# wedevxer/CUDA-AcceleratedVectorDatabaseEngine

Hardware: AMD Instinct MI355X
Metric: QPS + p99 latency, 10M×768D IVF-Flat k=10 nprobe=32, 1/2/4/8 MI355X (higher is better)
Workload: dtype fp32; 1 GPU; 10M x 768D IVF-Flat L2, nlist 4096, nprobe 32, batch 64, k 10; nvec=10000000, dim=768, nlist=4096, nprobe=32, batch=64, k=10, train_vectors=100000, parallelism=single GPU; 3 batches in flight

## Files before the change

cuda-acceleratedvectordatabaseengine_amd/csrc/screen.hip:

```cpp
#pragma clang fp contract(off)

#include <hip/hip_runtime.h>

#include <algorithm>
#include <stdexcept>
#include <cfloat>
#include <type_traits>

#include "kernels.hpp"
#include "scan_common.hpp"
#include "wave_topk.hpp"

namespace vdbk {

typedef __bf16 bf16x8 __attribute__((ext_vector_type(8)));
typedef float f32x4 __attribute__((ext_vector_type(4)));
typedef uint32_t u32x4 __attribute__((ext_vector_type(4)));
typedef int i32x4 __attribute__((ext_vector_type(4)));

constexpr float kScreenHuge = 1125899906842624.0f;
constexpr int kRing = 512;
#ifndef VDB_SCREEN_EXACT_PIPE
#define VDB_SCREEN_EXACT_PIPE 4
#endif
constexpr int kExactPipe = VDB_SCREEN_EXACT_PIPE;
#ifndef VDB_SCREEN_EXACT_PIPE_END
#define VDB_SCREEN_EXACT_PIPE_END 8
#endif
constexpr int kExactPipeEnd = VDB_SCREEN_EXACT_PIPE_END;
#ifndef VDB_SCREEN_DIAG
#define VDB_SCREEN_DIAG 0
#endif

__device__ __forceinline__ uint32_t bf16_bits(float f) {
    const uint32_t b = __float_as_uint(f);
    const uint32_t ex = b & 0x7F800000u;
    if (ex == 0) return 0u;
    if (ex == 0x7F800000u) return 0x7FC0u;
    return (b + 0x7FFFu + ((b >> 16) & 1u)) >> 16;
}
__device__ __forceinline__ float bf16_val(uint32_t h) { return __uint_as_float(h << 16); }

__device__ __forceinline__ uint4 pack_bf16x8(const float4 lo, const float4 hi) {
    uint4 r;
    r.x = bf16_bits(lo.x) | (bf16_bits(lo.y) << 16);
    r.y = bf16_bits(lo.z) | (bf16_bits(lo.w) << 16);
    r.z = bf16_bits(hi.x) | (bf16_bits(hi.y) << 16);
    r.w = bf16_bits(hi.z) | (bf16_bits(hi.w) << 16);
    return r;
}

__device__ __forceinline__ float4 resid(const float4 x, const float4 c) {
    return make_float4((float)((double)x.x - c.x), (float)((double)x.y - c.y), (float)((double)x.z - c.z),
                       (float)((double)x.w - c.w));
}

__device__ __forceinline__ float ru(double v) { return __double2float_ru(v * (1.0 + 0x1p-30)); }

__global__ __launch_bounds__(256) void ivf_screen_build(const float4* __restrict__ arena, uint64_t blocks,
                                                        uint32_t d4, const uint32_t* __restrict__ block_list,
                                                        const float* __restrict__ cent_rm, uint4* __restrict__ shadow,
                                                        float* __restrict__ rows, float4* __restrict__ meta) {
    const int lane = lane_id();
    const uint32_t dp = d4 * 4, ks = dp / 32;
    for (uint64_t b = (uint64_t)blockIdx.x * 4 + wave_index(); b < blocks; b += (uint64_t)gridDim.x * 4) {
        const float4* blk = arena + b * d4 * 64;
        const float4* cen = (const float4*)(cent_rm + (size_t)block_list[b] * dp);
        const uint64_t slot = b * 64 + lane;
        float4* row = rows ? (float4*)(rows + slot * dp) : nullptr;
        double x2 = 0.0, b2 = 0.0, e2 = 0.0;
        bool huge = false;
        for (uint32_t t = 0; t < d4; ++t) {
            const float4 x = blk[(size_t)t * 64 + lane];
            const float4 c = cen[t];
            if (rows) row[t] = x;
            const float xv[4] = {x.x, x.y, x.z, x.w}, cv[4] = {c.x, c.y, c.z, c.w};
#pragma unroll
            for (int i = 0; i < 4; ++i) {
                const double bd = (double)xv[i] - (double)cv[i];
                const double ed = bd - (double)bf16_val(bf16_bits((float)bd));
                huge |= !(fabs(bd) <= (double)kScreenHuge) || !(fabsf(xv[i]) <= kScreenHuge);
                x2 += (double)xv[i] * xv[i];
                b2 += bd * bd;
                e2 += ed * ed;
            }
        }
        meta[slot] = huge ? make_float4(__builtin_inff(), __builtin_inff(), __builtin_inff(), __builtin_inff())
                          : make_float4((float)b2, ru(sqrt(b2)), ru(sqrt(e2)), ru(sqrt(x2)));
        uint4* sh = shadow + b * (uint64_t)d4 * 32;
        const int vv = lane & 15, h = lane >> 4;
        for (uint32_t s = 0; s < ks; ++s) {
            const float4 c0 = cen[8 * s + 2 * h], c1 = cen[8 * s + 2 * h + 1];
            for (int vt = 0; vt < 4; ++vt) {
                const float4 lo = blk[(size_t)(8 * s + 2 * h) * 64 + 16 * vt + vv];
                const float4 hi = blk[(size_t)(8 * s + 2 * h + 1) * 64 + 16 * vt + vv];
                sh[((size_t)s * 4 + vt) * 64 + lane] = pack_bf16x8(resid(lo, c0), resid(hi, c1));
            }
        }
    }
}

template <int M>
__global__ __launch_bounds__(256) void ivf_screen_pairs(const float* __restrict__ q, uint32_t BP, uint32_t P,
                                                        const uint32_t* __restrict__ probes,
                                                        const float* __restrict__ cent_rm, uint32_t dp,
                                                        uint16_t* __restrict__ qres, float4* __restrict__ pst,
                                                        uint32_t* __restrict__ thr4, uint32_t* __restrict__ scnt,
                                                        uint32_t* __restrict__ ovf, uint32_t* __restrict__ counters,
                                                        uint32_t* __restrict__ ubcnt) {
    chain_prio();
    const int lane = lane_id();
    for (uint32_t e = blockIdx.x * blockDim.x + threadIdx.x; e < 4 * BP; e += gridDim.x * blockDim.x) thr4[e] = kThrInf;
    if (scnt)
        for (uint32_t e = blockIdx.x * blockDim.x + threadIdx.x; e < BP; e += gridDim.x * blockDim.x) {
            scnt[e] = 0u;
            ovf[e] = 0u;
            ubcnt[e] = 0u;
            if (e == 0) counters[kCtrCand] = counters[kCtrOvf] = counters[kCtrReal] = 0u;
        }
    for (uint32_t i = blockIdx.x * 4 + wave_index(); i < BP; i += gridDim.x * 4) {
        const float* qr = q + (size_t)(i / P) * dp;
        const float* cr = cent_rm + (size_t)probes[i] * dp;
        double a2 = 0.0, f2 = 0.0, c2 = 0.0, qc = 0.0;
        bool huge = false;
        for (uint32_t d = lane; d < dp; d += 64) {
            const float qv = qr[d], cv = cr[d];
            const double ad = M == kL2 ? (double)qv - (double)cv : (double)qv;
            const uint32_t h = bf16_bits((float)ad);
            qres[(size_t)i * dp + d] = (uint16_t)h;
            const double fd = ad - (double)bf16_val(h);
            huge |= !(fabs(ad) <= (double)kScreenHuge) || !(fabsf(qv) <= kScreenHuge) || !(fabsf(cv) <= kScreenHuge);
            a2 += ad * ad;
            f2 += fd * fd;
            c2 += (double)cv * cv;
            qc += (double)qv * cv;
        }
        for (int m = 32; m >= 1; m >>= 1) {
            a2 += __shfl_xor(a2, m);
            f2 += __shfl_xor(f2, m);
            c2 += __shfl_xor(c2, m);
            qc += __shfl_xor(qc, m);
        }
        huge = __ballot(huge) != 0;
        if (lane == 0) {
            const float inf = __builtin_inff();
            if (huge) pst[i] = make_float4(inf, inf, inf, inf);
            else if (M == kL2) pst[i] = make_float4((float)a2, ru(sqrt(a2)), ru(sqrt(f2)), 0.0f);
            else pst[i] = make_float4((float)qc, ru(sqrt(a2)), ru(sqrt(f2)), ru(sqrt(c2)));
        }
    }
}

__device__ __forceinline__ float i8_scale(float mx) { return mx > 0.0f ? mx * (1.0f / 127.0f) * (1.0f + 0x1p-20f) : 0.0f; }
__device__ __forceinline__ int i8_q(float r, float inv) { return max(-127, min(127, (int)rintf(r * inv))); }

__global__ __launch_bounds__(256) void ivf_screen_build_i8(const float4* __restrict__ arena, uint64_t blocks,
                                                           uint32_t d4, const uint32_t* __restrict__ block_list,
                                                           const float* __restrict__ cent_rm, uint4* __restrict__ shadow,
                                                           float* __restrict__ rows, float4* __restrict__ meta,
                                                           float* __restrict__ sscale) {
    const int lane = lane_id();
// ... 415 lines not shown
    char* base = (char*)slds + screen_item_lds(a.k, wq) + (size_t)wv * screen_wave_lds(a.k);
    uint64_t* tk_i = (uint64_t*)base;
    float* tk_d = (float*)(base + (size_t)16 * a.k * 8);
    float* kdl = tk_d + 16 * a.k;
    uint32_t* s_thr_w = (uint32_t*)(kdl + 16);
    uint32_t* ring = s_thr_w + 16;
    __shared__ uint32_t s_next, s_seg[2];
    __shared__ uint32_t s_thr[32];
    const int lane = lane_id();

    auto drain_narrow = [&]() {
        const uint32_t n_narrow = a.counters[0];
        for (;;) {
            uint32_t idx = 0;
            if (lane == 0) idx = atomicAdd(&a.work[0], 1u);
            idx = __builtin_amdgcn_readfirstlane(idx);
            if (idx >= n_narrow) break;
            ScanItem it = a.items[idx];
            it.list = __builtin_amdgcn_readfirstlane(it.list);
            it.seg = __builtin_amdgcn_readfirstlane(it.seg);
            it.pair_start = __builtin_amdgcn_readfirstlane(it.pair_start);
            it.npairs = __builtin_amdgcn_readfirstlane(it.npairs);
            if (lane < (int)it.npairs) s_thr_w[lane] = a.thr[it.pair_start + lane];
            __builtin_amdgcn_fence(__ATOMIC_RELEASE, "wavefront");
            screen_segment<M, KD>(a, it, 0, (int)it.npairs, it.seg, tk_d, tk_i, kdl, s_thr_w, ring, true, nullptr,
                                  it.seg);
            screen_partials(a, it, 0, (int)it.npairs, it.seg, tk_d, tk_i, true);
        }
    };

    const uint32_t n_wide = a.counters[3];
    uint32_t stride = a.wide_stride;
    if (stride > 1 && n_wide % stride == 0) stride = stride == 40009u ? 40013u : 40009u;
    if (a.fused && blockIdx.x + a.fused >= gridDim.x) drain_narrow();
    for (;;) {
        if (threadIdx.x == 0) s_next = atomicAdd(&a.work[1], 1u);
        __syncthreads();
        const uint32_t b = s_next;
        if (b >= n_wide) break;
        const uint32_t item = stride > 1 ? (uint32_t)(((uint64_t)b * stride) % n_wide) : b;
        ScanItem it = a.items_w[item];
        it.list = __builtin_amdgcn_readfirstlane(it.list);
        it.seg = __builtin_amdgcn_readfirstlane(it.seg);
        it.pair_start = __builtin_amdgcn_readfirstlane(it.pair_start);
        it.npairs = __builtin_amdgcn_readfirstlane(it.npairs);
        const int nq = (int)it.npairs;
        if (threadIdx.x < 2) s_seg[threadIdx.x] = 0;
        if (threadIdx.x < (uint32_t)nq) s_thr[threadIdx.x] = a.thr[it.pair_start + threadIdx.x];
        for (uint32_t e = threadIdx.x; e < (uint32_t)nq * a.k; e += blockDim.x) {
            it_d[e] = __builtin_inff();
            it_i[e] = kNoId;
        }
        if (threadIdx.x < (uint32_t)nq) {
            it_kd[threadIdx.x] = __builtin_inff();
            it_lock[threadIdx.x] = 0u;
        }
        __syncthreads();
        const uint32_t seg_vectors = a.seg_blocks * 64;
        const uint32_t nseg = (a.count[it.list] + seg_vectors - 1) / seg_vectors;
        const uint32_t seg0 = it.seg * a.segs_item, seg1 = min(nseg, seg0 + a.segs_item);
        const bool split = nq > 16;
        const uint32_t half = split ? wv >> 1 : 0u;
        const int nq0 = split ? (nq + 1) / 2 : nq;
        const int q0 = half ? nq0 : 0, nqh = half ? nq - nq0 : nq0;
        const int ko = q0 * (int)a.k;
        for (;;) {
            uint32_t sg = 0;
            if (lane == 0) sg = atomicAdd(&s_seg[half], 1u);
            sg = seg0 + __builtin_amdgcn_readfirstlane(sg);
            if (sg >= seg1) break;
            screen_segment<M, KD>(a, it, q0, nqh, sg, it_d + ko, it_i + ko, it_kd + q0, s_thr + q0, ring, false,
                                  it_lock + q0, it.seg);
            screen_partials(a, it, q0, nqh, sg, it_d + ko, it_i + ko, false);
        }
        __syncthreads();
        if ((wv & 1) == 0 && (wv == 0 || split)) screen_partials(a, it, q0, nqh, seg0, it_d + ko, it_i + ko, true);
    }
    if (a.fused) drain_narrow();
}


__device__ __forceinline__ void block_sort64(float (&u)[4]) {
    const int l = lane_id() & 15;
    bitonic64_step<2, 1>(u, l);
    bitonic64_step<4, 2>(u, l), bitonic64_step<4, 1>(u, l);
    bitonic64_step<8, 4>(u, l), bitonic64_step<8, 2>(u, l), bitonic64_step<8, 1>(u, l);
    bitonic64_step<16, 8>(u, l), bitonic64_step<16, 4>(u, l), bitonic64_step<16, 2>(u, l), bitonic64_step<16, 1>(u, l);
    bitonic64_step<32, 16>(u, l), bitonic64_step<32, 8>(u, l), bitonic64_step<32, 4>(u, l);
    bitonic64_step<32, 2>(u, l), bitonic64_step<32, 1>(u, l);
    bitonic64_step<64, 32>(u, l), bitonic64_step<64, 16>(u, l), bitonic64_step<64, 8>(u, l);
    bitonic64_step<64, 4>(u, l), bitonic64_step<64, 2>(u, l), bitonic64_step<64, 1>(u, l);
}
__device__ __forceinline__ void merge_sorted64(float (&rl)[4], const float (&u)[4]) {
    const int l = lane_id() & 15;
#pragma unroll
    for (int v = 0; v < 4; ++v) {
        const float rv = __uint_as_float((uint32_t)__builtin_amdgcn_mov_dpp((int)__float_as_uint(u[3 - v]), 0x140, 0xF,
                                                                            0xF, false));
        rl[v] = fminf(rl[v], rv);
    }
    bitonic64_step<64, 32>(rl, l), bitonic64_step<64, 16>(rl, l), bitonic64_step<64, 8>(rl, l);
    bitonic64_step<64, 4>(rl, l), bitonic64_step<64, 2>(rl, l), bitonic64_step<64, 1>(rl, l);
}
__device__ __forceinline__ float row_elem(const float (&u)[4], int e) {
    const int v = e & 3;
    const float x = v == 0 ? u[0] : v == 1 ? u[1] : v == 2 ? u[2] : u[3];
    return __shfl(x, (lane_id() & ~15) + (e >> 2));
}

struct CandChunk {
    uint32_t base = 0, left = 0;
    uint32_t next = 0;
    uint32_t real = 0;
    bool pending = false;
};
__device__ __forceinline__ void pad_cand(const ScanArgs& a, uint32_t base, uint32_t n) {
    for (uint32_t i = (uint32_t)lane_id(); i < n; i += 64)
        if (base + i < a.cand_cap) a.cand[base + i] = make_uint4(~0u, 0u, 0u, ~0u);
}
__device__ __forceinline__ void finish_cand(const ScanArgs& a, CandChunk& cc) {
    pad_cand(a, cc.base, cc.left);
    if (cc.pending) pad_cand(a, cc.next, kCandChunk);
    if (cc.real && lane_id() == 0) atomicAdd(a.ccount + (kCtrReal - kCtrCand), cc.real);
    cc.left = 0;
    cc.real = 0;
    cc.pending = false;
}

template <int M, int KD, int NG, bool I8, bool W2>
__device__ __forceinline__ void collect_segment(const ScanArgs& a, const ScanItem it, const int q0, const int nq,
                                                const uint32_t seg, float4* rl_lds, uint32_t* s_thr,
                                                const float4* s_pst, const float* s_qsc, float4* s_mt, float* s_vs,
                                                const uint32_t residue, CandChunk& cc) {
    const int lane = lane_id();
    const uint32_t dp = a.dp, ks = dp >> (I8 ? 6 : 5);
    const uint32_t count = a.count[it.list];
    const uint32_t seg_vectors = a.seg_blocks * 64;
    const uint64_t b0 = a.block_off[it.list] + (uint64_t)seg * a.seg_blocks;
    const uint32_t v0 = seg * seg_vectors;
    const uint32_t nv = min(count - v0, seg_vectors);
    const uint32_t nb = (nv + 63) >> 6;
    const int k = (int)a.k, kq = ((int)a.k + 3) / 4;
    const uint32_t* pairs = a.sorted_pair + it.pair_start + q0;
    const float cm = (float)(4 * dp + 16) * 0x1.02p-24f;
    const float cr = (float)(dp + 2) * 0x1.02p-24f;
    const float cu = 0x1.02p-23f;
    auto pair_of = [&](int g) -> uint32_t {
        const uint32_t pr = pairs[g];
        return (pr >> 16) * a.P + (pr & 0xFFFFu);
    };
    const uint4* qa_row[NG];
#pragma unroll
    for (int gg = 0; gg < NG; ++gg)
        qa_row[gg] = (const uint4*)((const char*)a.qres + (size_t)pair_of(min(16 * gg + (lane & 15), nq - 1)) * dp *
                                                              (I8 ? 1 : 2)) +
                     (lane >> 4);
    uint32_t collected = 0;
    float gthr[NG][4], gq4[NG][4];
#pragma unroll
    for (int gg = 0; gg < NG; ++gg)
#pragma unroll
        for (int r = 0; r < 4; ++r) gthr[gg][r] = gq4[gg][r] = __builtin_inff();
    const uint32_t thr_every = W2 ? a.thr_every : 1u;
    const uint32_t spl = it.pair_start + q0 + min(lane & (16 * NG - 1), nq - 1);

    const uint4* sp = a.shadow + b0 * (uint64_t)ks * 256 + lane;
    uint4 xa[KD][4], qa[NG][KD];
#pragma unroll
    for (int u = 0; u < KD; ++u) {
#pragma unroll
        for (int vt = 0; vt < 4; ++vt) xa[u][vt] = ld_nt_u4(sp + (size_t)(u * 4 + vt) * 64);
#pragma unroll
        for (int gg = 0; gg < NG; ++gg) qa[gg][u] = qa_row[gg][4 * (u % ks)];
    }
    using AccT = std::conditional_t<I8, i32x4, f32x4>;
    for (uint32_t j = 0; j < nb; ++j) {
        const uint64_t mslot = (b0 + j) * 64 + lane;
        const float4 mt_l = a.meta[mslot];
        float vs_l = 0.0f;
        if constexpr (I8) vs_l = a.sscale[mslot];
        const bool thr_now = j % thr_every == 0;
        uint32_t gt_l = 0u;
        uint4 t4_l = make_uint4(0u, 0u, 0u, 0u);
        if (thr_now) {
            gt_l = a.thr[spl];
            t4_l = *(const uint4*)(a.thr4 + (size_t)spl * 4);
        }
        const bool reserve = !cc.pending && cc.left < kCandChunk / 2;
        uint32_t reply = 0;
        if (reserve && lane == 0) reply = atomicAdd(a.ccount, kCandChunk);
        AccT acc[NG][4];
#pragma unroll
        for (int gg = 0; gg < NG; ++gg)
#pragma unroll
            for (int vt = 0; vt < 4; ++vt) acc[gg][vt] = AccT{0, 0, 0, 0};
        for (uint32_t s0 = 0; s0 < ks; s0 += KD) {
            static_for<0, KD>([&](auto uu) {
                constexpr int u = decltype(uu)::value;
#pragma unroll
                for (int gg = 0; gg < NG; ++gg) {
                    if constexpr (I8) {
                        const i32x4 A = as_i32x4(qa[gg][u]);
#pragma unroll
                        for (int vt = 0; vt < 4; ++vt)
                            acc[gg][vt] =
                                __builtin_amdgcn_mfma_i32_16x16x64_i8(A, as_i32x4(xa[u][vt]), acc[gg][vt], 0, 0, 0);
                    } else {
                        const bf16x8 A = as_bf16x8(qa[gg][u]);
#pragma unroll
                        for (int vt = 0; vt < 4; ++vt)
                            acc[gg][vt] =
                                __builtin_amdgcn_mfma_f32_16x16x32_bf16(A, as_bf16x8(xa[u][vt]), acc[gg][vt], 0, 0, 0);
                    }
                }
                const uint64_t nxt = (uint64_t)j * ks + s0 + u + KD;
#pragma unroll
                for (int vt = 0; vt < 4; ++vt) xa[u][vt] = ld_nt_u4(sp + (nxt * 4 + vt) * 64);
#pragma unroll
                for (int gg = 0; gg < NG; ++gg) qa[gg][u] = qa_row[gg][4 * ((s0 + u + KD) % ks)];
            });
        }
        s_mt[lane] = mt_l;
        if constexpr (I8) s_vs[lane] = vs_l;
        if (reserve) {
            cc.next = __builtin_amdgcn_readfirstlane(reply);
            cc.pending = true;
        }
        float gthr_l = 0.0f, gq4_l = 0.0f;
        if (thr_now) {
            const float th4 =
                fmaxf(fmaxf(ord_dec(t4_l.x), ord_dec(t4_l.y)), fmaxf(ord_dec(t4_l.z), ord_dec(t4_l.w)));
            gthr_l = fminf(ord_dec(gt_l), th4);
            gq4_l = ord_dec(residue == 0 ? t4_l.x : residue == 1 ? t4_l.y : residue == 2 ? t4_l.z : t4_l.w);
        }
        __builtin_amdgcn_fence(__ATOMIC_RELEASE, "wavefront");
#pragma unroll
        for (int gg = 0; gg < NG; ++gg) {
            const int g0 = 16 * gg;
            float ubv[4][4];
            float4 pst[4];
            float qsc[4];
#pragma unroll
            for (int r = 0; r < 4; ++r) {
                const int gc = min(g0 + 4 * (lane >> 4) + r, nq - 1);
                pst[r] = s_pst[gc];
                if constexpr (I8) qsc[r] = s_qsc[gc];
            }
#pragma unroll
            for (int vt = 0; vt < 4; ++vt) {
                const float4 mt = s_mt[16 * vt + (lane & 15)];
                float vsc = 0.0f;
                if constexpr (I8) vsc = s_vs[16 * vt + (lane & 15)];
                const bool valid = j * 64 + 16 * vt + (lane & 15) < nv;
#pragma unroll
                for (int r = 0; r < 4; ++r) {
                    float dot;
                    if constexpr (I8) dot = (float)acc[gg][vt][r] * (qsc[r] * vsc);
                    else dot = acc[gg][vt][r];
                    const float4 ps = pst[r];
                    const float approx = M == kL2 ? (ps.x + mt.x) - 2.0f * dot : -(ps.x + dot);
                    const float an = ps.y + ps.z, bn = mt.y + mt.z;
                    const float cs = an * mt.z + ps.z * bn + ps.z * mt.z;
                    float del;
                    if (M == kL2) {
                        const float rest = 2.0f * (cs + cm * (an * bn)) + cu * (ps.x + mt.x + fabsf(approx));
                        del = rest + cr * (fabsf(approx) + rest);
                    } else {
                        del = cs + cm * (an * bn) + cr * (ps.y * mt.w) + cu * (ps.y * ps.w + an * bn + fabsf(approx));
                    }
                    del = del * 1.001f + 1e-30f;
                    const float ub = approx + del;
                    if constexpr (I8) acc[gg][vt][r] = __float_as_int(approx - del);
                    else acc[gg][vt][r] = approx - del;
                    ubv[r][vt] = valid && ub == ub ? ub : __builtin_inff();
                }
            }
            float th[4], pub_t[4], pub_q[4];
#pragma unroll
            for (int r = 0; r < 4; ++r) {
                const int g = g0 + 4 * (lane >> 4) + r;
                const int gc = min(g, nq - 1);
                float4* rlp = rl_lds + (gg * 4 + r) * 64 + lane;
                const float4 rv = *rlp;
                float rl[4] = {rv.x, rv.y, rv.z, rv.w};
                float tw = row_elem(rl, k - 1), tq = row_elem(rl, kq - 1);
                if (thr_now) {
                    const float gn = __shfl(gthr_l, gc), qn = __shfl(gq4_l, gc);
                    if constexpr (W2) {
                        gthr[gg][r] = fminf(gthr[gg][r], gn);
                        gq4[gg][r] = fminf(gq4[gg][r], qn);
                    } else {
                        gthr[gg][r] = gn;
                        gq4[gg][r] = qn;
                    }
                }
                const float cur = fminf(gthr[gg][r], ord_dec(s_thr[gc]));
                const float bmin = fminf(fminf(ubv[r][0], ubv[r][1]), fminf(ubv[r][2], ubv[r][3]));
                if (__ballot(bmin < fminf(tw, cur))) {
                    block_sort64(ubv[r]);
                    merge_sorted64(rl, ubv[r]);
                    *rlp = make_float4(rl[0], rl[1], rl[2], rl[3]);
                    tw = row_elem(rl, k - 1);
                    tq = row_elem(rl, kq - 1);
                }
                pub_t[r] = tw < cur ? tw : __builtin_inff();
                pub_q[r] = tq < gq4[gg][r] ? tq : __builtin_inff();
                gthr[gg][r] = fminf(gthr[gg][r], tw);
                gq4[gg][r] = fminf(gq4[gg][r], tq);
                th[r] = g < nq ? fminf(tw, cur) : -__builtin_inff();
            }
            {
                const int lq = lane & 15, src = 16 * (lq >> 2), rs = lq & 3;
                float pt = __builtin_inff(), pq = __builtin_inff();
#pragma unroll
                for (int r = 0; r < 4; ++r) {
                    const float t = __shfl(pub_t[r], src), q = __shfl(pub_q[r], src);
                    if (rs == r) pt = t, pq = q;
                }
                if ((lane >> 4) == gg && g0 + lq < nq) {
                    if (pt < __builtin_inff()) {
                        atomicMin(&s_thr[g0 + lq], ord_enc(pt));
                        atomicMin(a.thr + spl, ord_enc(pt));
                    }
                    if (pq < __builtin_inff()) atomicMin(a.thr4 + (size_t)spl * 4 + residue, ord_enc(pq));
                }
            }
            auto lbv = [&](int vt, int r) -> float {
                if constexpr (I8) return __int_as_float(acc[gg][vt][r]);
                else return acc[gg][vt][r];
            };
            auto is_cand = [&](int vt, int r) {
                return j * 64 + 16 * vt + (lane & 15) < nv && g0 + 4 * (lane >> 4) + r < nq && !(lbv(vt, r) > th[r]);
            };
            uint32_t tot = 0;
#pragma unroll
            for (int vt = 0; vt < 4; ++vt)
#pragma unroll
                for (int r = 0; r < 4; ++r) tot += (uint32_t)__popcll(__ballot(is_cand(vt, r)));
            if (tot) {
                uint32_t cb0, cn0, cb1 = 0;
                if (tot <= cc.left) {
                    cb0 = cc.base;
                    cn0 = tot;
                    cc.base += tot;
                    cc.left -= tot;
                } else if (tot > kCandChunk) {
                    uint32_t v = 0;
                    if (lane == 0) v = atomicAdd(a.ccount, tot);
                    cb0 = __builtin_amdgcn_readfirstlane(v);
                    cn0 = tot;
                } else {
                    cb0 = cc.base;
                    cn0 = cc.left;
                    uint32_t v = 0;
                    if (cc.pending) {
                        cb1 = cc.next;
                        cc.pending = false;
                    } else {
                        if (lane == 0) v = atomicAdd(a.ccount, kCandChunk);
                        cb1 = __builtin_amdgcn_readfirstlane(v);
                    }
                    cc.base = cb1 + (tot - cn0);
                    cc.left = kCandChunk - (tot - cn0);
                }
                collected += tot;
                cc.real += tot;
                uint32_t rank = 0;
#pragma unroll
                for (int vt = 0; vt < 4; ++vt) {
#pragma unroll
                    for (int r = 0; r < 4; ++r) {
                        const bool c = is_cand(vt, r);
                        const uint64_t mm = __ballot(c);
                        if (c) {
                            const uint32_t rk = rank + __builtin_amdgcn_mbcnt_hi(
                                                           (uint32_t)(mm >> 32), __builtin_amdgcn_mbcnt_lo((uint32_t)mm, 0u));
                            const uint32_t idx = rk < cn0 ? cb0 + rk : cb1 + (rk - cn0);
                            const uint32_t spi = it.pair_start + q0 + g0 + 4 * (lane >> 4) + r;
                            const uint32_t slot = (uint32_t)((b0 + j) * 64 + 16 * vt + (lane & 15));
                            if (idx < a.cand_cap)
                                a.cand[idx] = make_uint4(spi, slot, __float_as_uint(lbv(vt, r)), 0u);
                            else {
                                a.ovf[spi] = 1u;
                                a.ccount[kCtrOvf - kCtrCand] = 1u;
                            }
                        }
                        rank += (uint32_t)__popcll(mm);
                    }
                }
            }
        }
    }
    if (a.mstats && lane == 0) {
        atomicAdd(&a.mstats[0], (unsigned long long)collected);
        atomicAdd(&a.mstats[1], (unsigned long long)nb);
    }
}

__device__ __forceinline__ void overflow_item(const ScanArgs& a, uint32_t pair_start, uint32_t npairs, uint32_t t0,
                                              uint32_t nt) {
    for (uint32_t t = t0; t < npairs; t += nt) a.ovf[pair_start + t] = 1u;
    if (t0 == 0) a.ccount[kCtrOvf - kCtrCand] = 1u;
}

__device__ __forceinline__ void reset_rl(float4* rl_lds, int rows) {
    const int lane = lane_id();
    const float inf = __builtin_inff();
    for (int r = 0; r < rows; ++r) rl_lds[r * 64 + lane] = make_float4(inf, inf, inf, inf);
}

__device__ __forceinline__ void contribute_rl(const ScanArgs& a, const ScanItem it, const int q0, const int nq,
                                              const float4* rl_lds) {
    const int lane = lane_id();
    const int k = (int)a.k;
    for (int r = 0; r < (nq + 15) / 16 * 4; ++r) {
        const int g = 16 * (r >> 2) + 4 * (lane >> 4) + (r & 3);
        const uint32_t spi = it.pair_start + q0 + min(g, nq - 1);
        uint32_t slot = 0;
        if ((lane & 15) == 0 && g < nq) slot = atomicAdd(&a.ubcnt[spi], 1u);
        slot = __shfl(slot, lane & ~15);
        const float4 rv = rl_lds[r * 64 + lane];
        const float rl[4] = {rv.x, rv.y, rv.z, rv.w};
        if (g < nq && slot < (uint32_t)kUbLists) {
            float* dst = a.ublist + ((size_t)spi * kUbLists + slot) * k;
#pragma unroll
            for (int v = 0; v < 4; ++v) {
                const int e = 4 * (lane & 15) + v;
                if (e < k) dst[e] = rl[v];
            }
        }
    }
}

__device__ __forceinline__ void put_stamp(const ScanArgs& a, uint64_t w0, uint64_t t0, uint64_t w3) {
    const uint32_t i = atomicAdd((unsigned int*)a.stamps, 1u);
    if (i < a.stamps_cap) {
        unsigned long long* r = a.stamps + 2 + (size_t)i * 4;
        r[0] = ((uint64_t)a.stamp_batch << 40) | w0;
        r[1] = t0;
        r[2] = wall_clock64();
        r[3] = w3;
    }
}

template <int M, int KD, bool W2, bool I8>
__global__ __launch_bounds__(256, W2 ? 1 : 2) void ivf_screen_collect(ScanArgs a) {
    __shared__ uint32_t s_next, s_seg;
    __shared__ uint32_t s_thr[32];
    __shared__ uint32_t s_thr_w[4][16];
    __shared__ float4 s_rl[4][8 * 64];
    __shared__ float4 s_pst[32], s_pst_w[4][16];
    __shared__ float s_qsc[32], s_qsc_w[4][16];
    __shared__ float4 s_mt[4][64];
    __shared__ float s_vs[4][64];
    const uint32_t wv = wave_index();
    const int lane = lane_id();
    float4* rl = s_rl[wv];
    CandChunk cc;
    auto pair_stats = [&](uint32_t ps, uint32_t t, float4* dp4, float* dsc) {
        const uint32_t pr = a.sorted_pair[ps + t];
        const uint32_t pi = (pr >> 16) * a.P + (pr & 0xFFFFu);
        dp4[t] = a.pst[pi];
        if (I8) dsc[t] = a.qscale[pi];
    };

    auto drain_narrow = [&]() {
        const uint32_t n_narrow = a.counters[0];
        for (;;) {
            uint32_t idx = 0;
            if (lane == 0) idx = atomicAdd(&a.work[0], 1u);
            idx = __builtin_amdgcn_readfirstlane(idx);
            if (idx >= n_narrow) break;
            ScanItem it = a.items[idx];
            it.list = __builtin_amdgcn_readfirstlane(it.list);
            it.seg = __builtin_amdgcn_readfirstlane(it.seg);
            it.pair_start = __builtin_amdgcn_readfirstlane(it.pair_start);
            it.npairs = __builtin_amdgcn_readfirstlane(it.npairs);
            if (it.npairs > 16u) {
                overflow_item(a, it.pair_start, it.npairs, (uint32_t)lane, 64u);
                continue;
            }
            if (lane < (int)it.npairs) {
                s_thr_w[wv][lane] = a.thr[it.pair_start + lane];
                pair_stats(it.pair_start, lane, s_pst_w[wv], s_qsc_w[wv]);
            }
            __builtin_amdgcn_fence(__ATOMIC_RELEASE, "wavefront");
            const uint64_t t0 = a.stamps ? wall_clock64() : 0;
            reset_rl(rl, 4);
            collect_segment<M, KD, 1, I8, W2>(a, it, 0, (int)it.npairs, it.seg, rl, s_thr_w[wv], s_pst_w[wv],
                                              s_qsc_w[wv], s_mt[wv], s_vs[wv], it.seg & 3u, cc);
            contribute_rl(a, it, 0, (int)it.npairs, rl);
            if (a.stamps && lane == 0)
                put_stamp(a, ((uint64_t)idx << 16) | blockIdx.x, t0, it.npairs | (1u << 8) | (1u << 16) | ((uint64_t)it.list << 32));
        }
    };

    const uint32_t n_wide = a.counters[3];
    if (a.stamps && threadIdx.x == 0) put_stamp(a, blockIdx.x, wall_clock64(), 2u << 16);
    if (a.fused && blockIdx.x + a.fused >= gridDim.x) drain_narrow();
    for (;;) {
        if (threadIdx.x == 0) s_next = atomicAdd(&a.work[1], 1u);
        __syncthreads();
        const uint32_t b = s_next;
        if (b >= n_wide) break;
        const uint64_t t_item = a.stamps ? wall_clock64() : 0;
        ScanItem it = a.items_w[b];
        it.list = __builtin_amdgcn_readfirstlane(it.list);
        it.seg = __builtin_amdgcn_readfirstlane(it.seg);
        it.pair_start = __builtin_amdgcn_readfirstlane(it.pair_start);
        it.npairs = __builtin_amdgcn_readfirstlane(it.npairs);
        const int nq = (int)it.npairs;
        if (nq > (W2 ? 32 : 16)) {
            overflow_item(a, it.pair_start, (uint32_t)nq, threadIdx.x, blockDim.x);
            __syncthreads();
            continue;
        }
        if (threadIdx.x == 0) s_seg = 0;
        if (threadIdx.x < (uint32_t)nq) {
            s_thr[threadIdx.x] = a.thr[it.pair_start + threadIdx.x];
            pair_stats(it.pair_start, threadIdx.x, s_pst, s_qsc);
        }
        __syncthreads();
        const uint32_t seg_vectors = a.seg_blocks * 64;
        const uint32_t nseg = (a.count[it.list] + seg_vectors - 1) / seg_vectors;
        const uint32_t seg0 = it.seg * a.segs_item, seg1 = min(nseg, seg0 + a.segs_item);
        reset_rl(rl, nq > 16 ? 8 : 4);
        bool any = false;
        for (;;) {
            uint32_t sg = 0;
            if (lane == 0) sg = atomicAdd(&s_seg, 1u);
            sg = seg0 + __builtin_amdgcn_readfirstlane(sg);
            if (sg >= seg1) break;
            if (W2 && nq > 16)
                collect_segment<M, KD, 2, I8, W2>(a, it, 0, nq, sg, rl, s_thr, s_pst, s_qsc, s_mt[wv], s_vs[wv], wv, cc);
            else
                collect_segment<M, KD, 1, I8, W2>(a, it, 0, nq, sg, rl, s_thr, s_pst, s_qsc, s_mt[wv], s_vs[wv], wv, cc);
            any = true;
        }
        if (any) contribute_rl(a, it, 0, nq, rl);
        __syncthreads();
        if (a.stamps && threadIdx.x == 0)
            put_stamp(a, ((uint64_t)b << 16) | blockIdx.x, t_item, (uint32_t)nq | ((seg1 - seg0) << 8) | ((uint64_t)it.list << 32));
    }
    if (a.fused) drain_narrow();
    finish_cand(a, cc);
}

bool scan_screen_fits(uint32_t k, uint32_t dp, uint32_t wq, bool deferred) {
    return k >= 1 && k <= 64 && dp % 64 == 0 && (wq == 16 || wq == 32) && screen_exact_lds(dp / 4) <= kLdsBytes / 2 &&
           (deferred || screen_item_lds(k, wq) + 4 * screen_wave_lds(k) + 256 <= kLdsBytes / 2);
}

size_t screen_shadow_u4(uint64_t blocks, uint32_t d4, bool i8) {
    return (size_t)(blocks + 2) * d4 * (i8 ? 16 : 32);
}

void launch_screen_build(const float4* arena, uint64_t blocks, uint32_t d4, const uint32_t* block_list,
                         const float* cent_rm, uint4* shadow, float* rows, float4* meta, hipStream_t s, float* sscale) {
    if (!blocks) return;
    const uint32_t g = (uint32_t)std::min<uint64_t>((blocks + 3) / 4, 8192);
    if (sscale) ivf_screen_build_i8<<<g, 256, 0, s>>>(arena, blocks, d4, block_list, cent_rm, shadow, rows, meta, sscale);
    else ivf_screen_build<<<g, 256, 0, s>>>(arena, blocks, d4, block_list, cent_rm, shadow, rows, meta);
}

void launch_screen_pairs(int metric, const float* q, uint32_t B, uint32_t P, const uint32_t* probes,
                         const float* cent_rm, uint32_t dp, uint16_t* qres, float4* pst, uint32_t* thr4, hipStream_t s,
                         uint32_t* scnt, uint32_t* ovf, uint32_t* counters, uint32_t* ubcnt, float* qscale) {
    const uint32_t BP = B * P;
    if (!BP) return;
    const uint32_t g = std::min<uint32_t>((BP + 3) / 4, 2048);
    if (qscale) {
        if (metric == kL2)
            ivf_screen_pairs_i8<kL2><<<g, 256, 0, s>>>(q, BP, P, probes, cent_rm, dp, (int8_t*)qres, qscale, pst, thr4,
                                                       scnt, ovf, counters, ubcnt);
        else
            ivf_screen_pairs_i8<kIP><<<g, 256, 0, s>>>(q, BP, P, probes, cent_rm, dp, (int8_t*)qres, qscale, pst, thr4,
                                                       scnt, ovf, counters, ubcnt);
        return;
    }
    if (metric == kL2)
        ivf_screen_pairs<kL2><<<g, 256, 0, s>>>(q, BP, P, probes, cent_rm, dp, qres, pst, thr4, scnt, ovf, counters, ubcnt);
    else
        ivf_screen_pairs<kIP><<<g, 256, 0, s>>>(q, BP, P, probes, cent_rm, dp, qres, pst, thr4, scnt, ovf, counters, ubcnt);
}

#ifndef VDB_COLLECT_KD
#define VDB_COLLECT_KD 4
#endif
void launch_screen_collect(int metric, uint32_t grid_blocks, const ScanArgs& a, hipStream_t s) {
    if (!grid_blocks) return;
    if (a.wide_q != 16 && a.wide_q != 32) throw std::length_error("launch_screen_collect: items of 16 or 32 queries only");
    const bool w2 = a.wide_q > 16;
    const uint32_t g = std::min<uint32_t>(grid_blocks, w2 ? kPersistentBlocks / 2 : kPersistentBlocks);
    auto go = [&](auto m_c, auto w_c, auto i_c) {
        constexpr int Mm = decltype(m_c)::value;
        constexpr bool Ww = decltype(w_c)::value;
        constexpr bool Ii = decltype(i_c)::value;
        constexpr int KW = Ii ? 6 : 8;
        const uint32_t ks = a.dp / (Ii ? 64 : 32);
        if (Ww && ks % KW == 0) ivf_screen_collect<Mm, KW, Ww, Ii><<<g, 256, 0, s>>>(a);
        else if (!Ww && VDB_COLLECT_KD != 4 && ks % VDB_COLLECT_KD == 0)
            ivf_screen_collect<Mm, VDB_COLLECT_KD, Ww, Ii><<<g, 256, 0, s>>>(a);
        else if (ks % 4 == 0) ivf_screen_collect<Mm, 4, Ww, Ii><<<g, 256, 0, s>>>(a);
        else if (ks % 2 == 0) ivf_screen_collect<Mm, 2, Ww, Ii><<<g, 256, 0, s>>>(a);
        else ivf_screen_collect<Mm, 1, Ww, Ii><<<g, 256, 0, s>>>(a);
    };
    auto go_w = [&](auto m_c, auto i_c) {
        if (w2) go(m_c, std::true_type{}, i_c);
        else go(m_c, std::false_type{}, i_c);
    };
    auto go_i = [&](auto m_c) {
        if (a.sscale) go_w(m_c, std::true_type{});
        else go_w(m_c, std::false_type{});
    };
    if (metric == kL2) go_i(std::integral_constant<int, kL2>{});
    else go_i(std::integral_constant<int, kIP>{});
}

void launch_scan_screen(int metric, uint32_t grid_blocks, const ScanArgs& a, hipStream_t s) {
    if (!grid_blocks) return;
    static const bool raised = [] {
        const void* f[] = {(const void*)ivf_scan_screen<kL2, 4>, (const void*)ivf_scan_screen<kL2, 2>,
                           (const void*)ivf_scan_screen<kIP, 4>, (const void*)ivf_scan_screen<kIP, 2>};
        for (const void* fn : f)
            (void)hipFuncSetAttribute(fn, hipFuncAttributeMaxDynamicSharedMemorySize, (int)(kLdsBytes / 2 - 256));
        (void)hipGetLastError();
        return true;
    }();
    (void)raised;
    const uint32_t g = std::min<uint32_t>(grid_blocks, kPersistentBlocks);
    const size_t lds = screen_item_lds(a.k, a.wide_q) + 4 * screen_wave_lds(a.k);
    const bool kd4 = (a.dp / 32) % 4 == 0;
    if (metric == kL2) {
        if (kd4) ivf_scan_screen<kL2, 4><<<g, 256, lds, s>>>(a);
        else ivf_scan_screen<kL2, 2><<<g, 256, lds, s>>>(a);
    } else {
        if (kd4) ivf_scan_screen<kIP, 4><<<g, 256, lds, s>>>(a);
        else ivf_scan_screen<kIP, 2><<<g, 256, lds, s>>>(a);
    }
}

}
```

Measured before the change: 47790 queries/s.

## Interleave query-to-row mapping so partial query groups skip unused screen rows

Remaps queries within each 16-query group so query i lands in row (i>>2) of lane group (i&3). A group with few queries then fills only the first few accumulator rows instead of spreading across all four. Bound computation, top-k merging, candidate ballots, row resets and contributions are skipped for unused rows, cutting wasted per-row work when nq is small. The change touches the MFMA operand load mapping, the threshold publication shuffles and the candidate indexing together. A mismatch in any of these would corrupt results, and the per-row guards add some branching.

After: 47540 queries/s. Within noise of the previous version (-0.5%).

```diff
diff --git a/cuda-acceleratedvectordatabaseengine_amd/csrc/collect_rows.hpp b/cuda-acceleratedvectordatabaseengine_amd/csrc/collect_rows.hpp
--- /dev/null
+++ b/cuda-acceleratedvectordatabaseengine_amd/csrc/collect_rows.hpp
@@ -0,0 +1,20 @@
+#pragma once
+
+#if defined(__HIPCC__) || defined(__CUDACC__)
+#define VDB_ROWS_FN __host__ __device__ inline constexpr
+#else
+#define VDB_ROWS_FN inline constexpr
+#endif
+
+namespace vdbrows {
+
+VDB_ROWS_FN int lane_group(int i) { return i & 3; }
+VDB_ROWS_FN int reg(int i) { return i >> 2; }
+VDB_ROWS_FN int row_of_query(int i) { return 4 * lane_group(i) + reg(i); }
+VDB_ROWS_FN int query_at(int h, int r) { return 4 * r + h; }
+VDB_ROWS_FN int query_of_row(int row) { return query_at(row >> 2, row & 3); }
+VDB_ROWS_FN int rows_used(int n) { return (n + 3) >> 2; }
+
+}
+
+#undef VDB_ROWS_FN
diff --git a/cuda-acceleratedvectordatabaseengine_amd/csrc/screen.hip b/cuda-acceleratedvectordatabaseengine_amd/csrc/screen.hip
--- a/cuda-acceleratedvectordatabaseengine_amd/csrc/screen.hip
+++ b/cuda-acceleratedvectordatabaseengine_amd/csrc/screen.hip
@@ -7,6 +7,7 @@
 #include <cfloat>
 #include <type_traits>
 
+#include "collect_rows.hpp"
 #include "kernels.hpp"
 #include "scan_common.hpp"
 #include "wave_topk.hpp"
@@ -728,7 +729,8 @@
     const uint4* qa_row[NG];
 #pragma unroll
     for (int gg = 0; gg < NG; ++gg)
-        qa_row[gg] = (const uint4*)((const char*)a.qres + (size_t)pair_of(min(16 * gg + (lane & 15), nq - 1)) * dp *
+        qa_row[gg] = (const uint4*)((const char*)a.qres +
+                                    (size_t)pair_of(min(16 * gg + vdbrows::query_of_row(lane & 15), nq - 1)) * dp *
                                                               (I8 ? 1 : 2)) +
                      (lane >> 4);
     uint32_t collected = 0;
@@ -813,106 +815,97 @@
 #pragma unroll
         for (int gg = 0; gg < NG; ++gg) {
             const int g0 = 16 * gg;
-            float ubv[4][4];
-            float4 pst[4];
-            float qsc[4];
+            const int nr = vdbrows::rows_used(min(nq - g0, 16));
+            const int lq = lane & 15, src = 16 * vdbrows::lane_group(lq), rs = vdbrows::reg(lq);
+            float pt = __builtin_inff(), pq = __builtin_inff();
+            float th[4];
 #pragma unroll
             for (int r = 0; r < 4; ++r) {
-                const int gc = min(g0 + 4 * (lane >> 4) + r, nq - 1);
-                pst[r] = s_pst[gc];
-                if constexpr (I8) qsc[r] = s_qsc[gc];
-            }
-#pragma unroll
-            for (int vt = 0; vt < 4; ++vt) {
-                const float4 mt = s_mt[16 * vt + (lane & 15)];
-                float vsc = 0.0f;
-                if constexpr (I8) vsc = s_vs[16 * vt + (lane & 15)];
-                const bool valid = j * 64 + 16 * vt + (lane & 15) < nv;
-#pragma unroll
-                for (int r = 0; r < 4; ++r) {
-                    float dot;
-                    if constexpr (I8) dot = (float)acc[gg][vt][r] * (qsc[r] * vsc);
-                    else dot = acc[gg][vt][r];
-                    const float4 ps = pst[r];
-                    const float approx = M == kL2 ? (ps.x + mt.x) - 2.0f * dot : -(ps.x + dot);
-                    const float an = ps.y + ps.z, bn = mt.y + mt.z;
-                    const float cs = an * mt.z + ps.z * bn + ps.z * mt.z;
-                    float del;
-                    if (M == kL2) {
-                        const float rest = 2.0f * (cs + cm * (an * bn)) + cu * (ps.x + mt.x + fabsf(approx));
-                        del = rest + cr * (fabsf(approx) + rest);
-                    } else {
-                        del = cs + cm * (an * bn) + cr * (ps.y * mt.w) + cu * (ps.y * ps.w + an * bn + fabsf(approx));
+                th[r] = -__builtin_inff();
+                if (r < nr) {
+                    const int g = g0 + vdbrows::query_at(lane >> 4, r);
+                    const int gc = min(g, nq - 1);
+                    const float4 ps = s_pst[gc];
+                    float qs = 0.0f;
+                    if constexpr (I8) qs = s_qsc[gc];
+                    float ub[4];
+#pragma unroll
+                    for (int vt = 0; vt < 4; ++vt) {
+                        const float4 mt = s_mt[16 * vt + (lane & 15)];
+                        float vsc = 0.0f;
+                        if constexpr (I8) vsc = s_vs[16 * vt + (lane & 15)];
+                        const bool valid = j * 64 + 16 * vt + (lane & 15) < nv;
+                        float dot;
+                        if constexpr (I8) dot = (float)acc[gg][vt][r] * (qs * vsc);
+                        else dot = acc[gg][vt][r];
+                        const float approx = M == kL2 ? (ps.x + mt.x) - 2.0f * dot : -(ps.x + dot);
+                        const float an = ps.y + ps.z, bn = mt.y + mt.z;
+                        const float cs = an * mt.z + ps.z * bn + ps.z * mt.z;
+                        float del;
+                        if (M == kL2) {
+                            const float rest = 2.0f * (cs + cm * (an * bn)) + cu * (ps.x + mt.x + fabsf(approx));
+                            del = rest + cr * (fabsf(approx) + rest);
+                        } else {
+                            del = cs + cm * (an * bn) + cr * (ps.y * mt.w) + cu * (ps.y * ps.w + an * bn + fabsf(approx));
+                        }
+                        del = del * 1.001f + 1e-30f;
+                        const float u = approx + del;
+                        if constexpr (I8) acc[gg][vt][r] = __float_as_int(approx - del);
+                        else acc[gg][vt][r] = approx - del;
+                        ub[vt] = valid && u == u ? u : __builtin_inff();
                     }
-                    del = del * 1.001f + 1e-30f;
-                    const float ub = approx + del;
-                    if constexpr (I8) acc[gg][vt][r] = __float_as_int(approx - del);
-                    else acc[gg][vt][r] = approx - del;
-                    ubv[r][vt] = valid && ub == ub ? ub : __builtin_inff();
+                    float4* rlp = rl_lds + (gg * 4 + r) * 64 + lane;
+                    const float4 rv = *rlp;
+                    float rl[4] = {rv.x, rv.y, rv.z, rv.w};
+                    float tw = row_elem(rl, k - 1), tq = row_elem(rl, kq - 1);
+                    if (thr_now) {
+                        const float gn = __shfl(gthr_l, gc), qn = __shfl(gq4_l, gc);
+                        if constexpr (W2) {
+                            gthr[gg][r] = fminf(gthr[gg][r], gn);
+                            gq4[gg][r] = fminf(gq4[gg][r], qn);
+                        } else {
+                            gthr[gg][r] = gn;
+                            gq4[gg][r] = qn;
+                        }
+                    }
+                    const float cur = fminf(gthr[gg][r], ord_dec(s_thr[gc]));
+                    const float bmin = fminf(fminf(ub[0], ub[1]), fminf(ub[2], ub[3]));
+                    if (__ballot(bmin < fminf(tw, cur))) {
+                        block_sort64(ub);
+                        merge_sorted64(rl, ub);
+                        *rlp = make_float4(rl[0], rl[1], rl[2], rl[3]);
+                        tw = row_elem(rl, k - 1);
+                        tq = row_elem(rl, kq - 1);
+                    }
+                    const float t = __shfl(tw < cur ? tw : __builtin_inff(), src);
+                    const float q = __shfl(tq < gq4[gg][r] ? tq : __builtin_inff(), src);
+                    if (rs == r) pt = t, pq = q;
+                    gthr[gg][r] = fminf(gthr[gg][r], tw);
+                    gq4[gg][r] = fminf(gq4[gg][r], tq);
+                    th[r] = g < nq ? fminf(tw, cur) : -__builtin_inff();
                 }
             }
-            float th[4], pub_t[4], pub_q[4];
-#pragma unroll
-            for (int r = 0; r < 4; ++r) {
-                const int g = g0 + 4 * (lane >> 4) + r;
-                const int gc = min(g, nq - 1);
-                float4* rlp = rl_lds + (gg * 4 + r) * 64 + lane;
-                const float4 rv = *rlp;
-                float rl[4] = {rv.x, rv.y, rv.z, rv.w};
-                float tw = row_elem(rl, k - 1), tq = row_elem(rl, kq - 1);
-                if (thr_now) {
-                    const float gn = __shfl(gthr_l, gc), qn = __shfl(gq4_l, gc);
-                    if constexpr (W2) {
-                        gthr[gg][r] = fminf(gthr[gg][r], gn);
-                        gq4[gg][r] = fminf(gq4[gg][r], qn);
-                    } else {
-                        gthr[gg][r] = gn;
-                        gq4[gg][r] = qn;
-                    }
+            if ((lane >> 4) == gg && g0 + lq < nq) {
+                if (pt < __builtin_inff()) {
+                    atomicMin(&s_thr[g0 + lq], ord_enc(pt));
+                    atomicMin(a.thr + spl, ord_enc(pt));
                 }
-                const float cur = fminf(gthr[gg][r], ord_dec(s_thr[gc]));
-                const float bmin = fminf(fminf(ubv[r][0], ubv[r][1]), fminf(ubv[r][2], ubv[r][3]));
-                if (__ballot(bmin < fminf(tw, cur))) {
-                    block_sort64(ubv[r]);
-                    merge_sorted64(rl, ubv[r]);
-                    *rlp = make_float4(rl[0], rl[1], rl[2], rl[3]);
-                    tw = row_elem(rl, k - 1);
-                    tq = row_elem(rl, kq - 1);
-                }
-                pub_t[r] = tw < cur ? tw : __builtin_inff();
-                pub_q[r] = tq < gq4[gg][r] ? tq : __builtin_inff();
-                gthr[gg][r] = fminf(gthr[gg][r], tw);
-                gq4[gg][r] = fminf(gq4[gg][r], tq);
-                th[r] = g < nq ? fminf(tw, cur) : -__builtin_inff();
-            }
-            {
-                const int lq = lane & 15, src = 16 * (lq >> 2), rs = lq & 3;
-                float pt = __builtin_inff(), pq = __builtin_inff();
-#pragma unroll
-                for (int r = 0; r < 4; ++r) {
-                    const float t = __shfl(pub_t[r], src), q = __shfl(pub_q[r], src);
-                    if (rs == r) pt = t, pq = q;
-                }
-                if ((lane >> 4) == gg && g0 + lq < nq) {
-                    if (pt < __builtin_inff()) {
-                        atomicMin(&s_thr[g0 + lq], ord_enc(pt));
-                        atomicMin(a.thr + spl, ord_enc(pt));
-                    }
-                    if (pq < __builtin_inff()) atomicMin(a.thr4 + (size_t)spl * 4 + residue, ord_enc(pq));
-                }
+                if (pq < __builtin_inff()) atomicMin(a.thr4 + (size_t)spl * 4 + residue, ord_enc(pq));
             }
             auto lbv = [&](int vt, int r) -> float {
                 if constexpr (I8) return __int_as_float(acc[gg][vt][r]);
                 else return acc[gg][vt][r];
             };
             auto is_cand = [&](int vt, int r) {
-                return j * 64 + 16 * vt + (lane & 15) < nv && g0 + 4 * (lane >> 4) + r < nq && !(lbv(vt, r) > th[r]);
+                return j * 64 + 16 * vt + (lane & 15) < nv && g0 + vdbrows::query_at(lane >> 4, r) < nq &&
+                       !(lbv(vt, r) > th[r]);
             };
             uint32_t tot = 0;
 #pragma unroll
             for (int vt = 0; vt < 4; ++vt)
 #pragma unroll
-                for (int r = 0; r < 4; ++r) tot += (uint32_t)__popcll(__ballot(is_cand(vt, r)));
+                for (int r = 0; r < 4; ++r)
+                    if (r < nr) tot += (uint32_t)__popcll(__ballot(is_cand(vt, r)));
             if (tot) {
                 uint32_t cb0, cn0, cb1 = 0;
                 if (tot <= cc.left) {
@@ -946,13 +939,14 @@
                 for (int vt = 0; vt < 4; ++vt) {
 #pragma unroll
                     for (int r = 0; r < 4; ++r) {
+                        if (r >= nr) continue;
                         const bool c = is_cand(vt, r);
                         const uint64_t mm = __ballot(c);
                         if (c) {
                             const uint32_t rk = rank + __builtin_amdgcn_mbcnt_hi(
                                                            (uint32_t)(mm >> 32), __builtin_amdgcn_mbcnt_lo((uint32_t)mm, 0u));
                             const uint32_t idx = rk < cn0 ? cb0 + rk : cb1 + (rk - cn0);
-                            const uint32_t spi = it.pair_start + q0 + g0 + 4 * (lane >> 4) + r;
+                            const uint32_t spi = it.pair_start + q0 + g0 + vdbrows::query_at(lane >> 4, r);
                             const uint32_t slot = (uint32_t)((b0 + j) * 64 + 16 * vt + (lane & 15));
                             if (idx < a.cand_cap)
                                 a.cand[idx] = make_uint4(spi, slot, __float_as_uint(lbv(vt, r)), 0u);
@@ -979,10 +973,14 @@
     if (t0 == 0) a.ccount[kCtrOvf - kCtrCand] = 1u;
 }
 
-__device__ __forceinline__ void reset_rl(float4* rl_lds, int rows) {
+__device__ __forceinline__ bool rl_row_used(int r, int nq) {
+    return (r & 3) < vdbrows::rows_used(min(nq - 16 * (r >> 2), 16));
+}
+__device__ __forceinline__ void reset_rl(float4* rl_lds, int nq) {
     const int lane = lane_id();
     const float inf = __builtin_inff();
-    for (int r = 0; r < rows; ++r) rl_lds[r * 64 + lane] = make_float4(inf, inf, inf, inf);
+    for (int r = 0; r < (nq + 15) / 16 * 4; ++r)
+        if (rl_row_used(r, nq)) rl_lds[r * 64 + lane] = make_float4(inf, inf, inf, inf);
 }
 
 __device__ __forceinline__ void contribute_rl(const ScanArgs& a, const ScanItem it, const int q0, const int nq,
@@ -990,7 +988,8 @@
     const int lane = lane_id();
     const int k = (int)a.k;
     for (int r = 0; r < (nq + 15) / 16 * 4; ++r) {
-        const int g = 16 * (r >> 2) + 4 * (lane >> 4) + (r & 3);
+        if (!rl_row_used(r, nq)) continue;
+        const int g = 16 * (r >> 2) + vdbrows::query_at(lane >> 4, r & 3);
         const uint32_t spi = it.pair_start + q0 + min(g, nq - 1);
         uint32_t slot = 0;
         if ((lane & 15) == 0 && g < nq) slot = atomicAdd(&a.ubcnt[spi], 1u);
@@ -1062,7 +1061,7 @@
             }
             __builtin_amdgcn_fence(__ATOMIC_RELEASE, "wavefront");
             const uint64_t t0 = a.stamps ? wall_clock64() : 0;
-            reset_rl(rl, 4);
+            reset_rl(rl, (int)it.npairs);
             collect_segment<M, KD, 1, I8, W2>(a, it, 0, (int)it.npairs, it.seg, rl, s_thr_w[wv], s_pst_w[wv],
                                               s_qsc_w[wv], s_mt[wv], s_vs[wv], it.seg & 3u, cc);
             contribute_rl(a, it, 0, (int)it.npairs, rl);
@@ -1100,7 +1099,7 @@
         const uint32_t seg_vectors = a.seg_blocks * 64;
         const uint32_t nseg = (a.count[it.list] + seg_vectors - 1) / seg_vectors;
         const uint32_t seg0 = it.seg * a.segs_item, seg1 = min(nseg, seg0 + a.segs_item);
-        reset_rl(rl, nq > 16 ? 8 : 4);
+        reset_rl(rl, nq);
         bool any = false;
         for (;;) {
             uint32_t sg = 0;
```
